# jinhan/tacotron2-vae

Measured on AMD Instinct MI355X. Metric: mel-frames/s (train step, batch=6, 80-mel), higher is better.
Workload: dtype f32; 1 GPU; configs[1]: Tacotron2-VAE fp32 train step (fwd+loss+bwd+clip+Adam), B=6/GPU fixed shape T_in=84 T_out=400, dropout on, random-init seed 1234; step_mode=hip-graph replay, decoder_forward=persistent, decoder_backward=persistent, startup_steps=43, global_batch=6, parallelism=dp1

## Files before the change

### include/t2vae.h

```cpp
#ifndef T2VAE_H
#define T2VAE_H
#include <stdint.h>
#ifdef __cplusplus
extern "C" {
#endif

#define T2V_OK 0
#define T2V_ERR_DIMS -1
#define T2V_ERR_ARG -2
#define T2V_ERR_LAUNCH -3

const char* t2v_version(void);
const char* t2v_last_error(void);

void t2v_set_phase_profile(unsigned long long* dev_buf32);
int t2v_stamp(unsigned long long* dev_buf, int slot, void* stream);
int t2v_debug_spin(int wgs, int microseconds, void* stream);

typedef struct t2v_step_params {
    uint64_t epoch;
    float lr;
    float bc1;
    float bc2s;
    float kl_weight;
// ... 213 lines not shown
int t2v_decoder_infer_steps_items(const t2v_dec_weights* w, const t2v_dec_infer_bufs* s, int B, int T_in,
                                  int t_begin, int t_end, float gate_threshold, float p_prenet,
                                  int external_prenet, uint64_t seed, const t2v_dec_items* items, void* stream);
int t2v_decoder_infer_persistent_items(const t2v_dec_persist_weights* w, const t2v_dec_persist_bufs* s, int B, int T_in,
                                       int t_end, float gate_threshold, float p_prenet, uint64_t seed,
                                       const t2v_dec_items* items, void* stream);

typedef struct t2v_dec_window {
    int32_t back;
    int32_t ahead;
} t2v_dec_window;
int t2v_decoder_infer_steps_window(const t2v_dec_weights* w, const t2v_dec_infer_bufs* s, int B, int T_in,
                                   int t_begin, int t_end, float gate_threshold, float p_prenet,
                                   int external_prenet, uint64_t seed, const t2v_dec_items* items,
                                   const t2v_dec_window* window, void* stream);
int t2v_decoder_infer_persistent_window(const t2v_dec_persist_weights* w, const t2v_dec_persist_bufs* s, int B, int T_in,
                                        int t_end, float gate_threshold, float p_prenet, uint64_t seed,
                                        const t2v_dec_items* items, const t2v_dec_window* window, void* stream);

int t2v_decoder_infer_steps_plan(const t2v_dec_weights* w, const t2v_dec_infer_bufs* s, int B, int T_in,
                                 int t_begin, int t_end, float gate_threshold, float p_prenet,
                                 int external_prenet, uint64_t seed, const t2v_dec_items* items,
                                 const t2v_dec_window* window, const int32_t* plan, int plan_stride, const int32_t* n_plan,
                                 void* stream);
int t2v_decoder_infer_persistent_plan(const t2v_dec_persist_weights* w, const t2v_dec_persist_bufs* s, int B, int T_in,
                                      int t_end, float gate_threshold, float p_prenet, uint64_t seed,
                                      const t2v_dec_items* items, const t2v_dec_window* window, const int32_t* plan,
                                      int plan_stride, const int32_t* n_plan, void* stream);

#define T2V_PLAN_MAX_SYMBOLS 4096
int t2v_duration_plan(const float* dur, int dur_stride, const int32_t* n_ids, const float* rate, int rate_stride_b,
                      int rate_stride_j, int B, int S, int T_max, int32_t* plan, int plan_stride, int32_t* n_plan,
                      void* stream);

int t2v_conv1d_stat_blocks(int B, int T, int Cin, int Cout, int KS);
int t2v_conv1d_stat_blocks_bf16(int B, int T, int Cin, int Cout, int KS);
long long t2v_conv1d_staged_launches(void);
int t2v_conv1d_fwd(const float* W, const float* X, const float* bias, float* Y, float* stat_part,
                   int B, int Cin, int T, int Cout, int KS, void* stream);
int t2v_conv1d_dw_scratch_floats(int B, int Cin, int T, int Cout, int KS);
int t2v_conv1d_bwd(const float* W, const float* X, const float* dY, float* dX, float* dW, float* Wt_scratch,
                   float* dw_scratch,
                   int B, int Cin, int T, int Cout, int KS, void* stream);
int t2v_conv1d_flip_weights(const float* const* W, float* const* Wt, const int* Cout, const int* Cin, int KS, int n,
                            void* stream);
int t2v_conv1d_fwd_bf16(const float* W, const float* X, const float* bias, float* Y, float* stat_part,
                        void* Wp_scratch, int B, int Cin, int T, int Cout, int KS, void* stream);
int t2v_conv1d_bwd_bf16(const float* W, const float* X, const float* dY, float* dX, float* dW,
                        void* Wp_scratch, float* dw_scratch, int B, int Cin, int T, int Cout, int KS, void* stream);

int t2v_bn_act_fwd(const float* y, const float* stat_part, int nblk, const float* gamma, const float* beta,
                   float* running_mean, float* running_var, float* mean_out, float* rstd_out, float* out,
                   int B, int M, int T, int act, int training, float p_drop, float momentum, float eps,
                   uint64_t seed, uint32_t rng_stream, uint32_t rng_t, void* stream);
int t2v_bn_act_fwd_len(const float* y, const float* gamma, const float* beta, const float* running_mean,
                       const float* running_var, float* out, const int32_t* lengths, int B, int M, int T, int act, float eps,
                       void* stream);
int t2v_bn_act_bwd(const float* y, const float* dout, const float* mean, const float* rstd,
                   const float* gamma, const float* beta, float* dy, float* dgamma, float* dbeta,
                   float* dconv_bias, int B, int M, int T, int act, float p_drop, uint64_t seed,
                   uint32_t rng_stream, uint32_t rng_t, void* stream);
int t2v_bn_act_bwd_eval(const float* y, const float* dout, const float* mean, const float* rstd,
                   const float* gamma, const float* beta, float* dy, float* dgamma, float* dbeta,
                   float* dconv_bias, int B, int M, int T, int act, float p_drop, uint64_t seed,
                   uint32_t rng_stream, uint32_t rng_t, void* stream);
int t2v_bn_act_slices(int backward, int B, int M, int T, int training, int has_partials);

int t2v_embedding_fwd(const long long* ids, const float* W, float* out_bct, int B, int T, int C, int n_symbols, void* stream);
int t2v_embedding_bwd(const long long* ids, const float* dy_bct, float* dW, int B, int T, int C, int n_symbols, void* stream);

int t2v_gemm_epilogue_bwd(const float* dy, const float* y, float* out, size_t n, float scale, void* stream);

long t2v_colsum_scratch_floats(long M, long N);
int t2v_colsum(const float* A, long lda, long M, long N, float* scratch, float* out, void* stream);

int t2v_mask_outputs(float* mel, float* mel_post, float* gate, const int* lengths, int B, int C, int T, float gate_fill,
                     void* stream);
int t2v_mask_time(const float* x, float* out, const int32_t* lengths, int B, int C, int T, void* stream);
int t2v_reparam_fwd(const float* eps, const float* mu, const float* logvar, float* z, long n, void* stream);
int t2v_reparam_bwd(const float* dz, const float* eps, const float* logvar, float* dlogvar, long n, void* stream);
int t2v_gather_words(const void* const* src, void* const* dst, int n, void* stream);
int t2v_concat2_rows(const float* a, long lda, int na, const float* b, long ldb, int nb, float* out, long rows, void* stream);

int t2v_bilstm_fwd(const float* gx, const float* whh, const int32_t* lengths, float* y, float* gates,
                   float* cells, float* hx_scratch, uint32_t* sync3, int B, int T, void* stream);
int t2v_bilstm_bwd(const float* whh, const int32_t* lengths, const float* dy, const float* gates,
                   const float* cells, float* dg, float* dgx_scratch, uint32_t* sync3, int B, int T,
                   void* stream);

int t2v_gemm_f32(const float* A, long sAi, long sAk, const float* B, long sBj, long sBk, const float* bias,
                 float* C, int ldc, int M, int N, int K, int relu, int accumulate, float p_drop,
                 uint64_t seed, uint32_t rng_stream, uint32_t rng_t, void* stream);
long t2v_gemm_splitk_scratch_floats(int M, int N, int K);
int t2v_gemm_f32_splitk(const float* A, long sAi, long sAk, const float* B, long sBj, long sBk, const float* bias,
                        float* C, int ldc, int M, int N, int K, int relu, int accumulate, float p_drop,
                        uint64_t seed, uint32_t rng_stream, uint32_t rng_t, float* splitk_scratch, void* stream);

int t2v_gemm_f32_set_mode(int x3);

typedef struct t2v_gemm_group {
    const float* A;
    long sAi;
    long sAk;
    int nb;
    const float* B[3];
    long sBj[3];
    long sBk[3];
    int N[3];
    float* C[3];
    int ldc[3];
} t2v_gemm_group;
long t2v_gemm_f32_grouped_scratch_floats(const t2v_gemm_group* groups, int ngroups, int M, int K);
int t2v_gemm_f32_grouped(const t2v_gemm_group* groups, int ngroups, int M, int K, int accumulate, float* scratch, void* stream);
long t2v_gemm_f32_grouped_group_offset(const t2v_gemm_group* groups, int ngroups, int M, int K, int g);
int t2v_gemm_f32_grouped_handed(const t2v_gemm_group* groups, int ngroups, int M, int K, int accumulate, float* scratch, int handed,
                                const uint32_t* done_ctr, int done_cap, void* stream);
long t2v_gemm_bf16_grouped_scratch_floats(const t2v_gemm_group* groups, int ngroups, int M, int K);
int t2v_gemm_bf16_grouped(const t2v_gemm_group* groups, int ngroups, int M, int K, int accumulate, float* scratch, void* stream);

int t2v_conv1d_x3_set_mode(int mode);
int t2v_conv1d_takes_x3(int B, int Cin, int T, int Cout, int KS, int bf16);
#define T2V_CONV_OP_FWD 0
#define T2V_CONV_OP_DX 1
#define T2V_CONV_OP_DW 2
#define T2V_CONV_ROUTE_GEMM 0
#define T2V_CONV_ROUTE_FWD 1
#define T2V_CONV_ROUTE_FWD_DMA 2
#define T2V_CONV_ROUTE_X3 3
#define T2V_CONV_ROUTE_BF16 4
#define T2V_CONV_ROUTE_BF16K32 5
#define T2V_CONV_ROUTE_PLANE1 6
#define T2V_CONV_ROUTE_DW 7
#define T2V_CONV_ROUTE_DW_BF16 8
#define T2V_CONV_ROUTES 9
int t2v_conv1d_route(int op, int B, int Cin, int T, int Cout, int KS, int bf16, int w_mod16, int* fallback, int* tile, int* ksplit,
                     int* dw_splits, int* stat_blocks, int* dw_scratch_floats, int* plane_splits, int* plane_chunk);
const char* t2v_conv1d_route_name(int route);

int t2v_gemm_f32_batched(const float* A, long sAb, long sAi, long sAk, const float* B, long sBb, long sBj, long sBk,
                         float* C, long sCb, int ldc, int nbatch, int M, int N, int K, void* stream);
int t2v_gemm_bf16(const float* A, long sAi, long sAk, const float* B, long sBj, long sBk, const float* bias,
                  float* C, int ldc, int M, int N, int K, int relu, int accumulate, float p_drop,
                  uint64_t seed, uint32_t rng_stream, uint32_t rng_t, void* stream);
long t2v_gemm_bf16_splitk_scratch_floats(int M, int N, int K);
int t2v_gemm_bf16_splitk(const float* A, long sAi, long sAk, const float* B, long sBj, long sBk, const float* bias,
                         float* C, int ldc, int M, int N, int K, int relu, int accumulate, float p_drop,
                         uint64_t seed, uint32_t rng_stream, uint32_t rng_t, float* splitk_scratch, void* stream);

#define T2V_GEMM_ROUTE_F32_64 0
#define T2V_GEMM_ROUTE_F32_64_SPLITK 1
#define T2V_GEMM_ROUTE_F32_BIG_128 2
#define T2V_GEMM_ROUTE_F32_BIG_64 3
#define T2V_GEMM_ROUTE_F32_X3 4
#define T2V_GEMM_ROUTE_BF16_64 5
#define T2V_GEMM_ROUTE_BF16_64_SPLITK 6
#define T2V_GEMM_ROUTE_BF16_BIG 7
#define T2V_GEMM_ROUTE_BF16_BIG_SPLITK 8
#define T2V_GEMM_ROUTE_BF16_PLANES 9
#define T2V_GEMM_ROUTE_BF16_TO_F32_BIG 10
#define T2V_GEMM_ROUTES 11
int t2v_gemm_route(int M, int N, int K, long sAi, long sAk, long sBj, long sBk, int a_mod16, int b_mod16, int scratch_mod16,
                   int has_scratch, int relu, float p_drop, int bf16, int* form, int* splits, int* k_per_split);
const char* t2v_gemm_route_name(int route);


int t2v_conv2d_s2_fwd(const float* x, const float* w, const float* bias, float* y, int B, int Cx, int H, int W,
// ... 181 lines not shown
```

### tacotron2-vae_amd/model.py

```python
from math import sqrt

import os

import torch
from torch import nn
from torch.nn import functional as F

import t2v_hip
from layers import ConvNorm, LinearNorm
from modules import VAE_GST
from utils import get_mask_from_lengths, to_gpu

drop_rate = 0.5
_drop_seed = [0x5EED]


class LocationLayer(nn.Module):
    def __init__(self, attention_n_filters, attention_kernel_size, attention_dim):
        super().__init__()
        self.location_conv = ConvNorm(2, attention_n_filters, kernel_size=attention_kernel_size,
                                      padding=(attention_kernel_size - 1) // 2, bias=False, stride=1,
                                      dilation=1)
        self.location_dense = LinearNorm(attention_n_filters, attention_dim, bias=False, w_init_gain='tanh')

# ... 297 lines not shown
        gate = s.GATE[:n].transpose(0, 1).unsqueeze(-1).contiguous()
        al = s.AL[1:n + 1].transpose(0, 1)
        if by_plan and min(pl[3]) < n:
            past = torch.arange(n, device=memory.device)[None, :] >= pl[1][:, None]
            mel = mel.masked_fill(past[:, None, :], 0.0)
            gate = gate.masked_fill(past[:, :, None], 1e3)
            al = al.masked_fill(past[:, :, None], 0.0)
        return mel, gate, al

    SEED_MASK = 0x7FFFFFFFFFFFFFFF

    def call_seed(self, call):
        return (int(self.dropout_seed) * 1000003 + int(call)) & self.SEED_MASK

    def reserve_seeds(self, n):
        seeds = [self.call_seed(self._calls + 1 + i) for i in range(n)]
        self._calls += n
        return seeds

    def inference_batch(self, memory, memory_lengths, seeds=None, chunk=32, persistent=None, plan=None, n_plan=None,
                        plan_window=(1, 1), plan_stop='plan'):
        B, T_in = memory.size(0), memory.size(1)
        lens = [int(x) for x in torch.as_tensor(memory_lengths).cpu().tolist()]
        if len(lens) != B or min(lens) < 1 or max(lens) > T_in:
            raise ValueError("memory_lengths must hold B = %d lengths in [1, %d]" % (B, T_in))
        if seeds is None:
            seeds = self.reserve_seeds(B)
        seeds = [int(x) for x in seeds]
        if len(seeds) != B:
            raise ValueError("seeds: %d seeds for %d utterances" % (len(seeds), B))
        pl = self._checked_plan(plan, n_plan, plan_window, plan_stop, B, memory.device)
        order = sorted(range(B), key=lambda b: -lens[b])
        items = [None] * B
        for g0 in range(0, B, 8):
            idx = order[g0:g0 + 8]
            L = max(lens[b] for b in idx)
            sel = torch.as_tensor(idx, device=memory.device)
            outs = self._decode_group(memory.index_select(0, sel)[:, :L].contiguous(), [lens[b] for b in idx],
                                      [seeds[b] for b in idx], chunk, persistent, self._plan_rows(pl, idx, memory.device))
            for b, o in zip(idx, outs):
                items[b] = o
        N = max(o[0].size(1) for o in items)
        mel = memory.new_zeros(B, self.n_mel_channels, N)
        gate = memory.new_full((B, N, 1), 1e3)
        al = memory.new_zeros(B, N, T_in)
        for b, (m, g, a) in enumerate(items):
            n = m.size(1)
            mel[b, :, :n] = m
            gate[b, :n, 0] = g
            al[b, :n, :a.size(1)] = a
        return mel, gate, al, torch.tensor([o[0].size(1) for o in items], dtype=torch.int64)

    def _decode_group(self, memory, lens, seeds, chunk, persistent, pl=None):
        lengths = torch.tensor(lens, dtype=torch.int32).to(memory.device)
        mask = torch.arange(memory.size(1), device=memory.device)[None, :] >= lengths[:, None]
        max_steps, thr = self._plan_steps(pl)
        s = self._session(memory, mask, max_steps, item_seeds=seeds, pl=pl)
        s.PRE[0].copy_(self.prenet(self.get_go_frame(memory)))
        self._run_to_end(s, chunk, persistent, 0, thr)
        if pl is not None and pl[4] == 'plan':
            return [(s.MEL[:n, j].t(), s.GATE[:n, j], s.AL[1:n + 1, j]) for j, n in enumerate(pl[3])]
        stops = s.stop_item.cpu().tolist()
        out = []
        for j, st in enumerate(stops):
            if st < s.max_steps:
                n = st + 1
            else:
                print("Warning! Reached max decoder steps")
                n = s.max_steps
            out.append((s.MEL[:n, j].t(), s.GATE[:n, j], s.AL[1:n + 1, j]))
        return out

    def _tf_rng_t(self):
        return self.__dict__.pop('_tf_t', None)

    def prepare(self, decoder_inputs):
        frames = self.parse_decoder_inputs(decoder_inputs)
        T = frames.size(0)
        x = torch.cat((frames.new_zeros(1, frames.size(1), frames.size(2)), frames[:T - 1]), 0)
        pre = self.prenet(x, self._tf_rng_t())
        att = self.attention_rnn
        gpre = t2v_hip.gemm(pre.detach().reshape(-1, pre.shape[-1]), att.weight_ih.detach()[:, :self.prenet_dim],
                            (att.bias_ih + att.bias_hh).detach())
        self._prepared = (decoder_inputs, pre, gpre, torch.cuda.current_stream(), self._param_operands())

    def _param_operands(self):
        dec = self.decoder_rnn
        return (dec.bias_ih + dec.bias_hh,
                torch.cat((self.linear_projection.weight, self.gate_layer.weight), 0),
                torch.cat((self.linear_projection.bias, self.gate_layer.bias), 0))

    def forward(self, memory, decoder_inputs, memory_lengths):
        B, T_in = memory.size(0), memory.size(1)
        prep = self.__dict__.pop('_prepared', None)
        gpre = None
        operands = None
        if prep is not None and prep[0] is decoder_inputs:
            _, pre, gpre, st, operands = prep
            T = pre.size(0)
            if st != torch.cuda.current_stream():
                torch.cuda.current_stream().wait_stream(st)
                for t in operands:
                    t.record_stream(torch.cuda.current_stream())
        else:
            frames = self.parse_decoder_inputs(decoder_inputs)
            T = frames.size(0)
            x = torch.cat((self.get_go_frame(memory).unsqueeze(0), frames), 0)
            pre = self.prenet(x[:T], self._tf_rng_t())
        att = self.attention_rnn
        lin = t2v_hip.LinearHIP.apply
        pm = lin(memory, self.attention_layer.memory_layer.weight, None, False, 0.0, 0, 0, 0)
        lengths = lengths_i32(memory_lengths, memory.device)
        training = self.training
        p_att = self.p_attention_dropout if training else 0.0
        p_dec = self.p_decoder_dropout if training else 0.0
        self._calls += 1
        seed = (int(self.dropout_seed) * 1000003 + self._calls) & 0x7FFFFFFFFFFFFFFF
        t2v_hip.stamp('dec_fwd_begin')
        b_dec, w81, b81 = operands if operands is not None else self._param_operands()
        hc, alignments = t2v_hip.DecoderCore.apply(None, memory, pm, lengths, *self._core_weights(b_dec),
                                                   p_att, p_dec, seed, torch.is_grad_enabled(),
                                                   pre, att.bias_ih, att.bias_hh, gpre)
        t2v_hip.stamp('dec_fwd_end')
        out = lin(hc, w81, b81, False, 0.0, 0, 0, 0)
        mel = out[..., :self.n_mel_channels].permute(1, 2, 0).contiguous()
        gate = out[..., self.n_mel_channels].transpose(0, 1).contiguous()
        return mel, gate, alignments


class SymbolEmbedding(nn.Embedding):

    def forward(self, ids):
        return t2v_hip.SymbolEmbedding.apply(ids, self.weight)


def lengths_i32(lengths, device):
    v = getattr(lengths, '_i32', None)
    if v is not None and v.device == device:
        return v
    return lengths.to(device=device, dtype=torch.int32)


class BatchLayout(object):
    _DT = (torch.int64, torch.int64, torch.float32, torch.float32, torch.int64, torch.float32, torch.float32)
    _ring = {}
    RING = 4
    n_symbols = None

    @classmethod
    def check_ids(cls, text):
        if cls.n_symbols is not None and text.numel() and not text.is_cuda:
            lo, hi = int(text.min()), int(text.max())
            if lo < 0 or hi >= cls.n_symbols:
                raise IndexError("symbol id out of range: got [%d, %d], embedding has %d rows" % (lo, hi, cls.n_symbols))

    def __init__(self, batch):
        self.check_ids(batch[0])
        self.max_len = int(torch.max(batch[1]).item())
        self.fields = []
        off = 0
        for t, dt in zip(batch, self._DT):
            nb = t.numel() * (8 if dt == torch.int64 else 4)
            self.fields.append((off, nb, dt, tuple(t.shape)))
            off += (nb + 15) & ~15
        self.i32 = []
        for idx in (1, 4):
            nb = batch[idx].numel() * 4
            self.i32.append((idx, off, nb))
            off += (nb + 15) & ~15
        self.nbytes = max(off, 16)
        self.key = tuple(f[3] for f in self.fields) + (self.max_len,)

    def pack_into(self, host, batch):
        for t, (off, nb, dt, shape) in zip(batch, self.fields):
            if nb:
                host[off:off + nb].view(dt).view(shape).copy_(t)
        for idx, off, nb in self.i32:
            if nb:
                host[off:off + nb].view(torch.int32).copy_(batch[idx].reshape(-1))

    def upload(self, batch, into=None):
        ring = self._ring.get(self.nbytes)
        if ring is None:
            ring = self._ring[self.nbytes] = [[torch.empty(self.nbytes, dtype=torch.uint8).pin_memory()
                                               for _ in range(self.RING)], [None] * self.RING, 0]
        slot = ring[2]
        ring[2] = (slot + 1) % self.RING
        if ring[1][slot] is not None:
            ring[1][slot].synchronize()
        host = ring[0][slot]
        self.pack_into(host, batch)
        dev = into if into is not None else torch.empty(self.nbytes, dtype=torch.uint8, device='cuda')
        assert dev.numel() == self.nbytes and dev.dtype == torch.uint8
        dev.copy_(host, non_blocking=True)
        ev = torch.cuda.Event()
        ev.record()
        ring[1][slot] = ev
        return dev

    def views(self, dev):
        v = [dev[off:off + nb].view(dt).view(shape) if nb else torch.empty(shape, dtype=dt, device=dev.device)
             for off, nb, dt, shape in self.fields]
        for idx, off, nb in self.i32:
            if nb:
                v[idx]._i32 = dev[off:off + nb].view(torch.int32)
        text, input_lengths, mel, gate, output_lengths, speakers, emotions = v
        return ((text, input_lengths, mel, self.max_len, output_lengths, speakers, emotions), (mel, gate))
# ... 108 lines not shown
```

### tacotron2-vae_amd/t2v_hip.py

```python
import collections
import ctypes as C
import math
import operator
import os

import torch

import t2v_abi

_HERE = os.path.dirname(os.path.abspath(__file__))
_LIB_PATH = os.environ.get('T2V_LIB') or os.path.join(_HERE, 'libt2vae_hip.so')
_lib = None

H, E, PRE, A, F_LOC, KS, XW, KATT, KATT_INF, G4 = 1024, 512, 256, 128, 32, 31, 2560, 1536, 1792, 4096

_ABI = t2v_abi.load()
T2VHipError = t2v_abi.T2VHipError

(_DecWeights, _DecTrainBufs, _DecBwdBufs, _DecPersistWeights, _DecPersistBufs, _DecTrainPersistWeights, _GemmGroup, _AchainDw,
 _DecInferBufs, _DecItems, _DecWindow) = (_ABI.classes[n] for n in (
     't2v_dec_weights', 't2v_dec_train_bufs', 't2v_dec_bwd_bufs', 't2v_dec_persist_weights', 't2v_dec_persist_bufs',
     't2v_dec_train_persist_weights', 't2v_gemm_group', 't2v_achain_dw', 't2v_dec_infer_bufs', 't2v_dec_items', 't2v_dec_window'))
_StepRecord = _ABI.classes['t2v_step_params']
if (_StepRecord.epoch.offset, _StepRecord.epoch.size) != (0, 8):
# ... 2826 lines not shown
                gemm(A, Bp, out=out, accumulate=accumulate)
        return
    arr = _group_array(groups)
    size_fn, run_fn = ((lib.t2v_gemm_bf16_grouped_scratch_floats, lib.t2v_gemm_bf16_grouped) if _BF16 else
                       (lib.t2v_gemm_f32_grouped_scratch_floats, lib.t2v_gemm_f32_grouped))
    nscr = size_fn(arr, len(groups), M, K)
    scr = torch.empty(max(nscr, 4), device=groups[0][0].device, dtype=torch.float32)
    _check(run_fn(arr, len(groups), M, K, int(bool(accumulate)), _p(scr), _stream()), 't2v_gemm_grouped')


def set_f32_gemm_mode(x3):
    return bool(load_library().t2v_gemm_f32_set_mode(-1 if x3 is None else int(bool(x3))))


def gemm(A, B, bias=None, out=None, relu=False, accumulate=False, p_drop=0.0, seed=0, rng_stream=0, rng_t=0):
    lib = _require_gpu(A, B)
    M, K = A.shape
    N, K2 = B.shape
    assert K == K2 and A.dtype == torch.float32 and B.dtype == torch.float32
    if out is None:
        out = torch.empty(M, N, device=A.device, dtype=torch.float32)
    assert out.shape == (M, N) and out.dtype == torch.float32 and (N == 1 or out.stride(1) == 1)
    ldc = out.stride(0) if M > 1 else max(N, out.stride(0))
    assert ldc >= N and (ldc == N or p_drop == 0.0)
    if True:
        nscr = lib.t2v_gemm_splitk_scratch_floats(M, N, K)
        if nscr and _BF16 and ((M + 63) // 64) * ((N + 63) // 64) >= 64:
            nscr = 0
        if nscr:
            scr = torch.empty(nscr, device=A.device, dtype=torch.float32)
            _check(lib.t2v_gemm_f32_splitk(_p(A), A.stride(0), A.stride(1), _p(B), B.stride(0), B.stride(1), _p(bias), _p(out),
                                           ldc, M, N, K, int(relu), int(accumulate), float(p_drop), int(seed), int(rng_stream),
                                           int(rng_t), _p(scr), _stream()), 't2v_gemm_f32_splitk')
            return out
    if _BF16:
        nscr = lib.t2v_gemm_bf16_splitk_scratch_floats(M, N, K)
        if nscr:
            scr = torch.empty(nscr, device=A.device, dtype=torch.float32)
            _check(lib.t2v_gemm_bf16_splitk(_p(A), A.stride(0), A.stride(1), _p(B), B.stride(0), B.stride(1), _p(bias), _p(out),
                                            ldc, M, N, K, int(relu), int(accumulate), float(p_drop), int(seed), int(rng_stream),
                                            int(rng_t), _p(scr), _stream()), 't2v_gemm_bf16_splitk')
            return out
    fn = lib.t2v_gemm_bf16 if _BF16 else lib.t2v_gemm_f32
    _check(fn(_p(A), A.stride(0), A.stride(1), _p(B), B.stride(0), B.stride(1), _p(bias), _p(out), ldc,
              M, N, K, int(relu), int(accumulate), float(p_drop), int(seed), int(rng_stream),
              int(rng_t), _stream()), 't2v_gemm_bf16' if _BF16 else 't2v_gemm_f32')
    return out


class LinearHIP(torch.autograd.Function):

    @staticmethod
    def forward(ctx, x, weight, bias, relu, p_drop, seed, rng_stream, rng_t):
        _require_gpu(x, weight)
        x2 = x.reshape(-1, x.shape[-1])
        x2 = x2 if x2.dtype == torch.float32 else x2.float()
        y = gemm(x2, weight, bias, relu=relu, p_drop=p_drop, seed=seed, rng_stream=rng_stream, rng_t=rng_t)
        ctx.save_for_backward(x2, weight, y if (relu or p_drop > 0) else None)
        ctx.cfg = (x.shape, bool(relu), float(p_drop), bias is not None)
        return y.view(*x.shape[:-1], weight.shape[0])

    @staticmethod
    def backward(ctx, dy):
        x2, weight, y = ctx.saved_tensors
        xshape, relu, p, has_bias = ctx.cfg
        dy2 = _f32c(dy.reshape(-1, weight.shape[0]))
        if relu or p > 0:
            scale = 1.0 / (1.0 - p) if p > 0 else 1.0
            masked = torch.empty_like(dy2)
            _check(load_library().t2v_gemm_epilogue_bwd(_p(dy2), _p(y), _p(masked), dy2.numel(), scale, _stream()),
                   't2v_gemm_epilogue_bwd')
            dy2 = masked
        fork = mark()
        dx = gemm(dy2, weight.t()) if ctx.needs_input_grad[0] else None
        if weight.is_leaf:
            with side('w', keep=(dy2, x2), after=fork):
                dw = gemm(dy2.t(), x2.t(), out=grad_slot(weight))
        else:
            dw = gemm(dy2.t(), x2.t())
        db = colsum(dy2) if has_bias else None
        return (dx.view(xshape) if dx is not None else None), dw, db, None, None, None, None, None


CONV2D_GEMM = os.environ.get('T2V_CONV2D_GEMM', '1') != '0'


class Conv2dBNReLU(torch.autograd.Function):

    @staticmethod
    def forward(ctx, x, weight, bias, gamma, beta, running_mean, running_var, training, coord):
        lib = _require_gpu(x, weight)
        x = _f32c(x)
        B, Cx, Hh, Ww = x.shape
        Cout = weight.shape[0]
        Ho, Wo = (Hh - 1) // 2 + 1, (Ww - 1) // 2 + 1
        f32 = dict(device=x.device, dtype=torch.float32)
        w = weight.contiguous()
        y = torch.empty(B, Cout, Ho, Wo, **f32)
        gscr = None
        if CONV2D_GEMM:
            gscr = torch.empty(lib.t2v_conv2d_s2_gemm_scratch_floats(B, Cx, Hh, Ww, Cout, int(coord)), **f32)
            _check(lib.t2v_conv2d_s2_fwd_gemm(_p(x), _p(w), _p(bias), _p(y), _p(gscr), B, Cx, Hh, Ww, Cout, int(coord), _stream()),
                   't2v_conv2d_s2_fwd_gemm')
        else:
            _check(lib.t2v_conv2d_s2_fwd(_p(x), _p(w), _p(bias), _p(y), B, Cx, Hh, Ww, Cout, int(coord), _stream()),
                   't2v_conv2d_s2_fwd')
        mean = torch.empty(Cout, **f32) if training else None
        rstd = torch.empty(Cout, **f32) if training else None
        out = torch.empty_like(y)
        _check(lib.t2v_bn_act_fwd(_p(y), None, 0, _p(gamma), _p(beta), _p(running_mean), _p(running_var), _p(mean),
                                  _p(rstd), _p(out), B, Cout, Ho * Wo, ACT_RELU, int(bool(training)), 0.0, 0.1, 1e-5,
                                  0, 0, 0, _stream()), 't2v_bn_act_fwd')
        ctx.keep = (x, w, y, mean, rstd, gamma, beta)
        ctx.gscr = gscr
        ctx.running = (running_mean, running_var)
        ctx.small = (gamma, beta, bias)
        ctx.cfg = (B, Cx, Hh, Ww, Cout, Ho, Wo, int(coord), bool(training))
        return out

    @staticmethod
    def backward(ctx, dout):
        lib = load_library()
        x, w, y, mean, rstd, gamma, beta = ctx.keep
        B, Cx, Hh, Ww, Cout, Ho, Wo, coord, training = ctx.cfg
        bn_bwd = lib.t2v_bn_act_bwd
        if not training:
            mean, rstd = ctx.running[0], torch.rsqrt(ctx.running[1] + 1e-5)
            bn_bwd = lib.t2v_bn_act_bwd_eval
        f32 = dict(device=x.device, dtype=torch.float32)
        dout = dout.contiguous()
        dy = torch.empty_like(y)
        dgamma, dbeta, dbias = _small_grads(ctx.small, Cout, f32)
        _check(bn_bwd(_p(y), _p(dout), _p(mean), _p(rstd), _p(gamma), _p(beta), _p(dy), _p(dgamma),
                      _p(dbeta), _p(dbias), B, Cout, Ho * Wo, ACT_RELU, 0.0, 0, 0, 0, _stream()), 't2v_bn_act_bwd')
        dx = torch.empty_like(x) if ctx.needs_input_grad[0] else None
        dw = torch.empty_like(w)
        if ctx.gscr is not None:
            _check(lib.t2v_conv2d_s2_bwd_gemm(_p(x), _p(w), _p(dy), _p(dx), _p(dw), _p(ctx.gscr), B, Cx, Hh, Ww, Cout, coord,
                                              _stream()), 't2v_conv2d_s2_bwd_gemm')
            ctx.gscr = None
        else:
            nscr = lib.t2v_conv2d_s2_dw_scratch_floats(B, Cx, Hh, Ww, Cout, coord)
            scr = torch.empty(nscr, **f32) if nscr else None
            _check(lib.t2v_conv2d_s2_bwd(_p(x), _p(w), _p(dy), _p(dx), _p(dw), _p(scr), B, Cx, Hh, Ww, Cout, coord,
                                         _stream()), 't2v_conv2d_s2_bwd')
        return dx, dw, dbias, dgamma, dbeta, None, None, None, None


class GRULast(torch.autograd.Function):

    @staticmethod
    def forward(ctx, x, w_ih, w_hh, b_ih, b_hh):
        lib = _require_gpu(x, w_ih)
        B, T, I = x.shape
        f32 = dict(device=x.device, dtype=torch.float32)
        x2 = _f32c(x).view(B * T, I)
        gi = gemm(x2, w_ih, b_ih)
        hs = torch.empty(B, T + 1, 256, **f32)
        gsave = torch.empty(B, T, 4, 256, **f32)
        whh = w_hh.contiguous()
        xchg = torch.empty(2 * 16 * 768, **f32)
        syncs = []
        gi3 = gi.view(B, T, 768)
        for b0 in range(0, B, MAX_DEC_B):
            b1 = min(B, b0 + MAX_DEC_B)
            sync = torch.empty(2, device=x.device, dtype=torch.int32)
# ... 200 lines not shown
```

Before: 231,300 mel-frames/s.

## Add fused native decoder output head kernels for mel/gate projection fwd and bwd

Replaces the generic linear GEMM plus permute/contiguous copies for the decoder mel and gate projection with dedicated MFMA kernels. The forward writes mel in (B, n_mel, T) layout and gate directly, and the backward computes d_hc, the weight grads and the bias grads without concatenating the weights or transposing activations. This removes torch.cat of the head weights, layout copies, and extra kernel launches, but adds split-K scratch plus a reduction pass for the weight gradients.

```diff
diff --git a/include/t2vae.h b/include/t2vae.h
--- a/include/t2vae.h
+++ b/include/t2vae.h
@@ -319,6 +319,14 @@
 int t2v_gather_words(const void* const* src, void* const* dst, int n, void* stream);
 int t2v_concat2_rows(const float* a, long lda, int na, const float* b, long ldb, int nb, float* out, long rows, void* stream);
 
+int t2v_dec_head_fwd(const float* hc, const float* W_proj, const float* b_proj, const float* W_gate, const float* b_gate,
+                     float* mel, float* gate, int T, int B, int K, int n_mel, void* stream);
+int t2v_dec_head_bwd_dx(const float* d_mel, const float* d_gate, const float* W_proj, const float* W_gate, float* d_hc,
+                        int T, int B, int K, int n_mel, void* stream);
+long t2v_dec_head_bwd_dw_scratch_floats(int T, int B, int K, int n_mel);
+int t2v_dec_head_bwd_dw(const float* d_mel, const float* d_gate, const float* hc, float* scratch, float* dW_proj, float* db_proj,
+                        float* dW_gate, float* db_gate, int T, int B, int K, int n_mel, void* stream);
+
 int t2v_bilstm_fwd(const float* gx, const float* whh, const int32_t* lengths, float* y, float* gates,
                    float* cells, float* hx_scratch, uint32_t* sync3, int B, int T, void* stream);
 int t2v_bilstm_bwd(const float* whh, const int32_t* lengths, const float* dy, const float* gates,
diff --git a/tacotron2-vae_amd/csrc/dec_head.hip b/tacotron2-vae_amd/csrc/dec_head.hip
--- /dev/null
+++ b/tacotron2-vae_amd/csrc/dec_head.hip
@@ -0,0 +1,251 @@
+#include "t2v_common.h"
+#include "t2v_kernels.h"
+
+#define DH_CT 6
+#define DH_NCMAX (16 * DH_CT)
+#define DH_SLICES 24
+
+__device__ __forceinline__ const float* dh_wrow(const float* __restrict__ Wp, const float* __restrict__ Wg, int c, int n_mel, int K) {
+    return c < n_mel ? Wp + (size_t)c * K : (c == n_mel ? Wg : nullptr);
+}
+__device__ __forceinline__ float dh_dy(const float* __restrict__ d_mel, const float* __restrict__ d_gate, int b, int c, int t,
+                                       int n_mel, int T) {
+    if (t >= T) return 0.f;
+    if (c < n_mel) return d_mel ? d_mel[((size_t)b * n_mel + c) * T + t] : 0.f;
+    return (c == n_mel && d_gate) ? d_gate[(size_t)b * T + t] : 0.f;
+}
+
+__device__ __forceinline__ float4 dh_ld4(const float* p, bool ok) {
+    float4 v = {0.f, 0.f, 0.f, 0.f};
+    if (ok) v = *(const float4*)p;
+    return v;
+}
+
+#define DH_FW 8
+__global__ __launch_bounds__(64 * DH_FW) void k_dec_head_fwd(const float* __restrict__ hc, const float* __restrict__ Wp,
+                                                             const float* __restrict__ bp, const float* __restrict__ Wg,
+                                                             const float* __restrict__ bg, float* __restrict__ mel, float* __restrict__ gate,
+                                                             int T, int B, int K, int n_mel) {
+    const int tid = threadIdx.x, lane = tid & 63, w = tid >> 6, li = lane & 15, g = lane >> 4;
+    const int b = blockIdx.y, t0 = 16 * blockIdx.x, t = t0 + li;
+    const int nkb = (K + 15) / 16, per = (nkb + DH_FW - 1) / DH_FW, kb0 = w * per, kb1 = min(nkb, kb0 + per);
+    const float* arow = t < T ? hc + ((size_t)t * B + b) * K : nullptr;
+    const float* wrow[DH_CT];
+#pragma unroll
+    for (int ct = 0; ct < DH_CT; ++ct) wrow[ct] = dh_wrow(Wp, Wg, 16 * ct + li, n_mel, K);
+    f32x4 acc[DH_CT][4];
+#pragma unroll
+    for (int ct = 0; ct < DH_CT; ++ct)
+#pragma unroll
+        for (int j = 0; j < 4; ++j) acc[ct][j] = f32x4{0.f, 0.f, 0.f, 0.f};
+    float4 a, bw[DH_CT];
+    {
+        const int k = 16 * kb0 + 4 * g;
+        const bool kin = kb0 < kb1 && k < K;
+        a = dh_ld4(arow + k, kin && arow);
+#pragma unroll
+        for (int ct = 0; ct < DH_CT; ++ct) bw[ct] = dh_ld4(wrow[ct] + k, kin && wrow[ct]);
+    }
+    for (int kb = kb0; kb < kb1; ++kb) {
+        const int k = 16 * (kb + 1) + 4 * g;
+        const bool kin = kb + 1 < kb1 && k < K;
+        const float4 an = dh_ld4(arow + k, kin && arow);
+        float4 bn[DH_CT];
+#pragma unroll
+        for (int ct = 0; ct < DH_CT; ++ct) bn[ct] = dh_ld4(wrow[ct] + k, kin && wrow[ct]);
+#pragma unroll
+        for (int ct = 0; ct < DH_CT; ++ct) {
+            acc[ct][0] = mfma16x4(a.x, bw[ct].x, acc[ct][0]);
+            acc[ct][1] = mfma16x4(a.y, bw[ct].y, acc[ct][1]);
+            acc[ct][2] = mfma16x4(a.z, bw[ct].z, acc[ct][2]);
+            acc[ct][3] = mfma16x4(a.w, bw[ct].w, acc[ct][3]);
+        }
+        a = an;
+#pragma unroll
+        for (int ct = 0; ct < DH_CT; ++ct) bw[ct] = bn[ct];
+    }
+    __shared__ float red[DH_FW][DH_NCMAX][17];
+#pragma unroll
+    for (int ct = 0; ct < DH_CT; ++ct)
+#pragma unroll
+        for (int r = 0; r < 4; ++r) red[w][16 * ct + li][4 * g + r] = (acc[ct][0][r] + acc[ct][1][r]) + (acc[ct][2][r] + acc[ct][3][r]);
+    __syncthreads();
+    const int NC = n_mel + 1;
+    for (int o = tid; o < 16 * NC; o += 64 * DH_FW) {
+        const int c = o >> 4, i = o & 15;
+        if (t0 + i >= T) continue;
+        const float s = ((red[0][c][i] + red[1][c][i]) + (red[2][c][i] + red[3][c][i])) +
+                        ((red[4][c][i] + red[5][c][i]) + (red[6][c][i] + red[7][c][i]));
+        if (c < n_mel) mel[((size_t)b * n_mel + c) * T + t0 + i] = s + bp[c];
+        else gate[(size_t)b * T + t0 + i] = s + bg[0];
+    }
+}
+
+#define DH_XW 4
+__global__ __launch_bounds__(64 * DH_XW) void k_dec_head_bwd_dx(const float* __restrict__ d_mel, const float* __restrict__ d_gate,
+                                                                const float* __restrict__ Wp, const float* __restrict__ Wg,
+                                                                float* __restrict__ d_hc, int T, int B, int K, int n_mel) {
+    const int tid = threadIdx.x, lane = tid & 63, w = tid >> 6, li = lane & 15, g = lane >> 4;
+    const int b = blockIdx.y, t0 = 16 * blockIdx.x;
+    const int ns = (n_mel + 1 + 3) / 4;
+    float a[DH_NCMAX / 4];
+#pragma unroll
+    for (int s = 0; s < DH_NCMAX / 4; ++s) a[s] = s < ns ? dh_dy(d_mel, d_gate, b, 4 * s + g, t0 + li, n_mel, T) : 0.f;
+    const int ncb = (K + 63) / 64;
+    for (int cb = w; cb < ncb; cb += DH_XW) {
+        const int n = 64 * cb + 4 * li;
+        const bool nin = n < K;
+        f32x4 acc[4][4];
+#pragma unroll
+        for (int q = 0; q < 4; ++q)
+#pragma unroll
+            for (int j = 0; j < 4; ++j) acc[q][j] = f32x4{0.f, 0.f, 0.f, 0.f};
+#pragma unroll
+        for (int s = 0; s < DH_NCMAX / 4; ++s) {
+            if (s < ns) {
+                const float* wr = dh_wrow(Wp, Wg, 4 * s + g, n_mel, K);
+                const float4 bw = dh_ld4(wr + n, nin && wr);
+                acc[s & 3][0] = mfma16x4(a[s], bw.x, acc[s & 3][0]);
+                acc[s & 3][1] = mfma16x4(a[s], bw.y, acc[s & 3][1]);
+                acc[s & 3][2] = mfma16x4(a[s], bw.z, acc[s & 3][2]);
+                acc[s & 3][3] = mfma16x4(a[s], bw.w, acc[s & 3][3]);
+            }
+        }
+#pragma unroll
+        for (int r = 0; r < 4; ++r) {
+            const int t = t0 + 4 * g + r;
+            float v[4];
+#pragma unroll
+            for (int j = 0; j < 4; ++j) v[j] = (acc[0][j][r] + acc[1][j][r]) + (acc[2][j][r] + acc[3][j][r]);
+            if (nin && t < T) *(float4*)(d_hc + ((size_t)t * B + b) * K + n) = float4{v[0], v[1], v[2], v[3]};
+        }
+    }
+}
+
+__global__ __launch_bounds__(256) void k_dec_head_dw(const float* __restrict__ d_mel, const float* __restrict__ d_gate,
+                                                     const float* __restrict__ hc, float* __restrict__ part, int T, int B, int K, int n_mel,
+                                                     int tiles_per_slice) {
+    const int tid = threadIdx.x, lane = tid & 63, w = tid >> 6, li = lane & 15, g = lane >> 4;
+    const int n = 64 * (4 * blockIdx.x + w) + 4 * li;
+    const bool nin = n < K;
+    const int nt = (T + 15) / 16, ntiles = nt * B;
+    const int c0 = blockIdx.y * tiles_per_slice, c1 = min(ntiles, c0 + tiles_per_slice);
+    f32x4 acc[DH_CT][4];
+#pragma unroll
+    for (int ct = 0; ct < DH_CT; ++ct)
+#pragma unroll
+        for (int j = 0; j < 4; ++j) acc[ct][j] = f32x4{0.f, 0.f, 0.f, 0.f};
+    for (int ch = c0; ch < c1; ++ch) {
+        const int b = ch / nt, t0 = 16 * (ch - b * nt);
+#pragma unroll
+        for (int q = 0; q < 4; ++q) {
+            const int t = t0 + 4 * q + g;
+            const float4 x = dh_ld4(hc + ((size_t)t * B + b) * K + n, nin && t < T);
+            float a[DH_CT];
+#pragma unroll
+            for (int ct = 0; ct < DH_CT; ++ct) a[ct] = dh_dy(d_mel, d_gate, b, 16 * ct + li, t, n_mel, T);
+#pragma unroll
+            for (int ct = 0; ct < DH_CT; ++ct) {
+                acc[ct][0] = mfma16x4(a[ct], x.x, acc[ct][0]);
+                acc[ct][1] = mfma16x4(a[ct], x.y, acc[ct][1]);
+                acc[ct][2] = mfma16x4(a[ct], x.z, acc[ct][2]);
+                acc[ct][3] = mfma16x4(a[ct], x.w, acc[ct][3]);
+            }
+        }
+    }
+    const int NC = n_mel + 1;
+    if (!nin) return;
+#pragma unroll
+    for (int ct = 0; ct < DH_CT; ++ct)
+#pragma unroll
+        for (int r = 0; r < 4; ++r) {
+            const int c = 16 * ct + 4 * g + r;
+            if (c < NC)
+                *(float4*)(part + ((size_t)blockIdx.y * NC + c) * K + n) = float4{acc[ct][0][r], acc[ct][1][r], acc[ct][2][r], acc[ct][3][r]};
+        }
+}
+
+__global__ __launch_bounds__(256) void k_dec_head_dw_sum(const float* __restrict__ part, int slices, const float* __restrict__ d_mel,
+                                                         const float* __restrict__ d_gate, float* __restrict__ dWp, float* __restrict__ dbp,
+                                                         float* __restrict__ dWg, float* __restrict__ dbg, int T, int B, int K, int n_mel,
+                                                         int nwb) {
+    const int tid = threadIdx.x, NC = n_mel + 1, K4 = K / 4;
+    if ((int)blockIdx.x < nwb) {
+        const int e = blockIdx.x * 256 + tid;
+        if (e >= NC * K4) return;
+        const int c = e / K4, k = 4 * (e - c * K4);
+        float4 s = *(const float4*)(part + (size_t)c * K + k);
+        for (int y = 1; y < slices; ++y) {
+            const float4 v = *(const float4*)(part + ((size_t)y * NC + c) * K + k);
+            s.x += v.x; s.y += v.y; s.z += v.z; s.w += v.w;
+        }
+        float* o = c < n_mel ? dWp + (size_t)c * K + k : dWg + k;
+        o[0] = s.x; o[1] = s.y; o[2] = s.z; o[3] = s.w;
+        return;
+    }
+    const int c = blockIdx.x - nwb;
+    __shared__ float red[256];
+    float s = 0.f;
+    for (int i = tid; i < B * T; i += 256) {
+        const int b = i / T;
+        s += dh_dy(d_mel, d_gate, b, c, i - b * T, n_mel, T);
+    }
+    red[tid] = s;
+    __syncthreads();
+    for (int h = 128; h > 0; h >>= 1) {
+        if (tid < h) red[tid] += red[tid + h];
+        __syncthreads();
+    }
+    if (tid == 0) { if (c < n_mel) dbp[c] = red[0]; else dbg[0] = red[0]; }
+}
+
+static bool dh_shape_ok(int T, int B, int K, int n_mel) {
+    return T >= 1 && B >= 1 && B <= 65535 && K >= 4 && !(K & 3) && n_mel >= 1 && n_mel + 1 <= DH_NCMAX &&
+           (long)T * B * K <= 0x7fffffffL * 4 && (T + 15) / 16 <= 0x7fffffff / B;
+}
+static bool dh_al16(const void* p) { return !((uintptr_t)p & 15); }
+static int dh_slices(int T, int B, int* tiles_per_slice) {
+    const int ntiles = (T + 15) / 16 * B;
+    const int want = ntiles < DH_SLICES ? ntiles : DH_SLICES;
+    const int per = (ntiles + want - 1) / want;
+    if (tiles_per_slice) *tiles_per_slice = per;
+    return (ntiles + per - 1) / per;
+}
+
+extern "C" int t2v_dec_head_fwd(const float* hc, const float* W_proj, const float* b_proj, const float* W_gate, const float* b_gate,
+                                float* mel, float* gate, int T, int B, int K, int n_mel, void* stream_) {
+    if (!hc || !W_proj || !b_proj || !W_gate || !b_gate || !mel || !gate || !dh_shape_ok(T, B, K, n_mel) || !dh_al16(hc) ||
+        !dh_al16(W_proj) || !dh_al16(W_gate)) return T2V_ERR_ARG;
+    k_dec_head_fwd<<<dim3((unsigned)((T + 15) / 16), (unsigned)B), 64 * DH_FW, 0, (hipStream_t)stream_>>>(hc, W_proj, b_proj, W_gate, b_gate, mel,
+                                                                                                 gate, T, B, K, n_mel);
+    return t2v_check_launch();
+}
+
+extern "C" int t2v_dec_head_bwd_dx(const float* d_mel, const float* d_gate, const float* W_proj, const float* W_gate, float* d_hc,
+                                   int T, int B, int K, int n_mel, void* stream_) {
+    if (!W_proj || !W_gate || !d_hc || !dh_shape_ok(T, B, K, n_mel) || !dh_al16(d_hc) || !dh_al16(W_proj) || !dh_al16(W_gate))
+        return T2V_ERR_ARG;
+    k_dec_head_bwd_dx<<<dim3((unsigned)((T + 15) / 16), (unsigned)B), 64 * DH_XW, 0, (hipStream_t)stream_>>>(d_mel, d_gate, W_proj, W_gate, d_hc,
+                                                                                                    T, B, K, n_mel);
+    return t2v_check_launch();
+}
+
+extern "C" long t2v_dec_head_bwd_dw_scratch_floats(int T, int B, int K, int n_mel) {
+    if (!dh_shape_ok(T, B, K, n_mel)) return 0;
+    return (long)dh_slices(T, B, nullptr) * (n_mel + 1) * K;
+}
+
+extern "C" int t2v_dec_head_bwd_dw(const float* d_mel, const float* d_gate, const float* hc, float* scratch, float* dW_proj,
+                                   float* db_proj, float* dW_gate, float* db_gate, int T, int B, int K, int n_mel, void* stream_) {
+    if (!hc || !scratch || !dW_proj || !db_proj || !dW_gate || !db_gate || !dh_shape_ok(T, B, K, n_mel) || !dh_al16(hc) ||
+        !dh_al16(scratch)) return T2V_ERR_ARG;
+    hipStream_t stream = (hipStream_t)stream_;
+    int per = 1;
+    const int slices = dh_slices(T, B, &per);
+    if ((long)slices * (n_mel + 1) * K > 0x7fffffffL) return T2V_ERR_ARG;
+    k_dec_head_dw<<<dim3((unsigned)((K + 255) / 256), (unsigned)slices), 256, 0, stream>>>(d_mel, d_gate, hc, scratch, T, B, K, n_mel, per);
+    const int nwb = ((n_mel + 1) * (K / 4) + 255) / 256;
+    k_dec_head_dw_sum<<<(unsigned)(nwb + n_mel + 1), 256, 0, stream>>>(scratch, slices, d_mel, d_gate, dW_proj, db_proj, dW_gate, db_gate,
+                                                                      T, B, K, n_mel, nwb);
+    return t2v_check_launch();
+}
diff --git a/tacotron2-vae_amd/model.py b/tacotron2-vae_amd/model.py
--- a/tacotron2-vae_amd/model.py
+++ b/tacotron2-vae_amd/model.py
@@ -403,11 +403,21 @@
         att = self.attention_rnn
         gpre = t2v_hip.gemm(pre.detach().reshape(-1, pre.shape[-1]), att.weight_ih.detach()[:, :self.prenet_dim],
                             (att.bias_ih + att.bias_hh).detach())
-        self._prepared = (decoder_inputs, pre, gpre, torch.cuda.current_stream(), self._param_operands())
+        self._prepared = (decoder_inputs, pre, gpre, torch.cuda.current_stream(),
+                          (self._dec_bias(),) if self._head_native() else self._param_operands())
+
+    def _head_params(self):
+        return (self.linear_projection.weight, self.linear_projection.bias, self.gate_layer.weight, self.gate_layer.bias)
+
+    def _head_native(self):
+        return t2v_hip.dec_head_native(*self._head_params())
+
+    def _dec_bias(self):
+        dec = self.decoder_rnn
+        return dec.bias_ih + dec.bias_hh
 
     def _param_operands(self):
-        dec = self.decoder_rnn
-        return (dec.bias_ih + dec.bias_hh,
+        return (self._dec_bias(),
                 torch.cat((self.linear_projection.weight, self.gate_layer.weight), 0),
                 torch.cat((self.linear_projection.bias, self.gate_layer.bias), 0))
 
@@ -438,12 +448,18 @@
         self._calls += 1
         seed = (int(self.dropout_seed) * 1000003 + self._calls) & 0x7FFFFFFFFFFFFFFF
         t2v_hip.stamp('dec_fwd_begin')
-        b_dec, w81, b81 = operands if operands is not None else self._param_operands()
+        native = self._head_native()
+        if operands is None or (not native and len(operands) != 3):
+            operands = (self._dec_bias(),) if native else self._param_operands()
+        b_dec = operands[0]
         hc, alignments = t2v_hip.DecoderCore.apply(None, memory, pm, lengths, *self._core_weights(b_dec),
                                                    p_att, p_dec, seed, torch.is_grad_enabled(),
                                                    pre, att.bias_ih, att.bias_hh, gpre)
         t2v_hip.stamp('dec_fwd_end')
-        out = lin(hc, w81, b81, False, 0.0, 0, 0, 0)
+        if native:
+            mel, gate = t2v_hip.DecoderHead.apply(hc, *self._head_params())
+            return mel, gate, alignments
+        out = lin(hc, operands[1], operands[2], False, 0.0, 0, 0, 0)
         mel = out[..., :self.n_mel_channels].permute(1, 2, 0).contiguous()
         gate = out[..., self.n_mel_channels].transpose(0, 1).contiguous()
         return mel, gate, alignments
diff --git a/tacotron2-vae_amd/t2v_hip.py b/tacotron2-vae_amd/t2v_hip.py
--- a/tacotron2-vae_amd/t2v_hip.py
+++ b/tacotron2-vae_amd/t2v_hip.py
@@ -2932,6 +2932,70 @@
         return (dx.view(xshape) if dx is not None else None), dw, db, None, None, None, None, None
 
 
+DEC_HEAD = os.environ.get('T2V_DEC_HEAD', '1') != '0'
+DEC_HEAD_MAX_ROWS = 96
+
+
+def dec_head_native(w_proj, b_proj, w_gate, b_gate):
+    if not DEC_HEAD or _BF16:
+        return False
+    ts = (w_proj, b_proj, w_gate, b_gate)
+    if not all(t.is_cuda and t.dtype == torch.float32 and t.is_contiguous() for t in ts):
+        return False
+    n_mel, K = w_proj.shape
+    return (K >= 4 and K % 4 == 0 and n_mel + 1 <= DEC_HEAD_MAX_ROWS and tuple(w_gate.shape) == (1, K) and b_proj.numel() == n_mel and
+            b_gate.numel() == 1 and w_proj.data_ptr() % 16 == 0 and w_gate.data_ptr() % 16 == 0)
+
+
+class DecoderHead(torch.autograd.Function):
+
+    @staticmethod
+    def forward(ctx, hc, w_proj, b_proj, w_gate, b_gate):
+        lib = _require_gpu(hc, w_proj, w_gate)
+        hc = _f32c(hc)
+        T, B, K = hc.shape
+        n_mel = w_proj.shape[0]
+        mel = torch.empty(B, n_mel, T, device=hc.device, dtype=torch.float32)
+        gate = torch.empty(B, T, device=hc.device, dtype=torch.float32)
+        _check(lib.t2v_dec_head_fwd(_p(hc), _p(w_proj), _p(b_proj), _p(w_gate), _p(b_gate), _p(mel), _p(gate), T, B, K, n_mel,
+                                    _stream()), 't2v_dec_head_fwd')
+        ctx.save_for_backward(hc, w_proj, b_proj, w_gate, b_gate)
+        ctx.set_materialize_grads(False)
+        return mel, gate
+
+    @staticmethod
+    def backward(ctx, d_mel, d_gate):
+        lib = load_library()
+        hc, w_proj, b_proj, w_gate, b_gate = ctx.saved_tensors
+        T, B, K = hc.shape
+        n_mel = w_proj.shape[0]
+        d_mel = None if d_mel is None else _f32c(d_mel)
+        d_gate = None if d_gate is None else _f32c(d_gate)
+        f32 = dict(device=hc.device, dtype=torch.float32)
+        fork = mark()
+        d_hc = None
+        if ctx.needs_input_grad[0]:
+            d_hc = torch.empty(T, B, K, **f32)
+            _check(lib.t2v_dec_head_bwd_dx(_p(d_mel), _p(d_gate), _p(w_proj), _p(w_gate), _p(d_hc), T, B, K, n_mel, _stream()),
+                   't2v_dec_head_bwd_dx')
+        params = (w_proj, b_proj, w_gate, b_gate)
+
+        def wgrads():
+            out = [grad_slot(p) for p in params]
+            out = [torch.empty(p.shape, **f32) if g is None else g for g, p in zip(out, params)]
+            scr = torch.empty(lib.t2v_dec_head_bwd_dw_scratch_floats(T, B, K, n_mel), **f32)
+            _check(lib.t2v_dec_head_bwd_dw(_p(d_mel), _p(d_gate), _p(hc), _p(scr), *(_p(g) for g in out), T, B, K, n_mel, _stream()),
+                   't2v_dec_head_bwd_dw')
+            return out
+
+        if all(p.is_leaf for p in params):
+            with side('w', keep=(d_mel, d_gate, hc), after=fork):
+                grads = wgrads()
+        else:
+            grads = wgrads()
+        return (d_hc, *grads)
+
+
 CONV2D_GEMM = os.environ.get('T2V_CONV2D_GEMM', '1') != '0'
 
 
```

Result: no change. 232,800 mel-frames/s, median of 6 (+0.7%).
